# ubisoft/ubisoft-laforge-ZeroEGGS

Measured on AMD Instinct MI355X. Metric: train_frames_per_sec, higher is better.
Workload: dtype f32; 1 GPU; configs_v1.json nets (25.5M params, random-init), batch 32/GPU x 256-frame windows from synthetic 60fps 2-min clips, style example 384 frames, full train step (gather+fwd+loss+bwd+allreduce+RAdam); global_batch=32, window=256, parallelism=dp1

## Files before the change

### include/zeggs_hip.h

```cpp
#ifndef ZEGGS_HIP_H
#define ZEGGS_HIP_H
#include <stddef.h>
#include <stdint.h>

#ifdef __cplusplus
extern "C" {
#endif

int zeggs_version(void);
const char* zeggs_last_error(void);
int zeggs_set_option(const char* name, int value);
int zeggs_timing_ms(int which, float* ms);

int zeggs_gemm(const float* A, const float* B, float* C, const float* bias, int M, int N, int K,
               long sam, long sak, long sbk, long sbn, long scm, long scn, int nbatch, long bsA,
               long bsB, long bsC, float alpha, float beta, int act, void* stream);
int zeggs_gemm_tn_bias(const float* dy, long lddy, const float* x, long ldx, float* dW, long lddw, int M_contract, int N, int K,
                       float beta, float* db, void* stream);
int zeggs_gemm_direct_selftest(int big, int depth, int shield);
int zeggs_gemm_direct_state(int big, int depth, int shield);
int zeggs_gemm_direct_warm(void);
int zeggs_gemm_route(int direct, int shield, int depth, int reserve);
int zeggs_gemm_route_get(int* out4);
int zeggs_gemm_kbatch(const float* A, const float* B, float* C, int M, int N, int K, long sam, long sak, long sbk, long sbn,
// ... 136 lines not shown
int zeggs_decoder_bwd(const ZeggsDecDims*, const ZeggsDecParams*, const ZeggsDecStats*, const float* gaze,
                      const float* pose, const float* rpos, const float* rrot, const float* dpose,
                      const float* drpos, const float* drrot, const ZeggsDecGrads*, float* dspeech,
                      float* dstyle, void* ws, size_t ws_bytes, void* stream);
#define ZEGGS_STATUS_WORDS 4
#define ZEGGS_GAVE_UP_DECODE 1u
#define ZEGGS_GAVE_UP_TRAIN_FWD 2u
#define ZEGGS_GAVE_UP_BPTT 4u
#define ZEGGS_GAVE_UP_BATCH_FWD 8u
typedef struct {
  int prepared;
  int defer_wgrads;
  void* wgrad_stream;
  unsigned* status;
  int grads_zeroed;
} ZeggsDecCall;
int zeggs_decoder_fwd_ex(const ZeggsDecDims*, const ZeggsDecParams*, const ZeggsDecStats*, const float* pose0,
                         const float* rpos0, const float* rrot0, const float* gaze, const float* speech,
                         const float* style, float* pose, float* rpos, float* rrot, int training, void* ws,
                         size_t ws_bytes, void* stream, const ZeggsDecCall* call);
int zeggs_decoder_bwd_ex(const ZeggsDecDims*, const ZeggsDecParams*, const ZeggsDecStats*, const float* gaze,
                         const float* pose, const float* rpos, const float* rrot, const float* dpose,
                         const float* drpos, const float* drrot, const ZeggsDecGrads*, float* dspeech,
                         float* dstyle, void* ws, size_t ws_bytes, void* stream, const ZeggsDecCall* call);
int zeggs_decoder_fwd_state_ex(const ZeggsDecDims*, const ZeggsDecParams*, const ZeggsDecStats*, const float* pose0,
                               const float* rpos0, const float* rrot0, const float* gaze, const float* speech,
                               const float* style, float* pose, float* rpos, float* rrot, const float* h_in,
                               float* h_out, void* ws, size_t ws_bytes, void* stream, const ZeggsDecCall* call);
size_t zeggs_decoder_batch_workspace_bytes(const ZeggsDecDims*);
int zeggs_decoder_batch_prepare(const ZeggsDecDims*, const ZeggsDecParams*, const ZeggsDecStats*, void* ws, size_t ws_bytes,
// ... 201 lines not shown
```

### ubisoft-laforge-zeroeggs_amd/csrc/decoder.hip

```cpp
#include "../../include/zeggs_hip.h"
#include "common.h"
#include "gemm.h"
#include "kernels.h"
#include "dec_math.h"
#include "dec_prologue.h"
#include "decoder_ws.h"

int g_decoder_fast = 1;
int g_bwd_chunks = 1;
int g_tp_prologue = 1;
int g_wgrad_order = 0;

extern "C" int zeggs_persistent_state(int which ) {
  return g_sweep_kernels[which == 0 ? SWEEP_DECODE : which == 1 ? SWEEP_ROLLOUT : SWEEP_BPTT].state;
}

namespace {

__global__ void dec_init_k(ZeggsDecDims d, ZeggsDecStats st, const float* pose0, const float* rp0, const float* rr0,
                           const float* gaze, const float* style, float* pose, float* rpos, float* rrot,
                           float* cse_in, float* gin1, int GL) {
  dec_init_body(blockIdx.x, d, st, pose0, rp0, rr0, gaze, style, pose, rpos, rrot, cse_in, gin1, GL);
}

__global__ void dec_fill_cond_k(ZeggsDecDims d, const float* speech, const float* style, float* gin, int GL, int t0,
                                int nt, long slot_stride, int ring) {
// ... 117 lines not shown
    dst[b * ldd + c] = src[b * lds + off + c];
  }
}

__global__ void dec_scatter_cond_grad_k(ZeggsDecDims d, const float* DX, int XD, float* dspeech, float* dstyle) {
  const int XC = d.SP + (d.film ? 0 : d.ST);
  long n = (long)d.T * d.B * XC;
  for (long i = (long)blockIdx.x * blockDim.x + threadIdx.x; i < n; i += (long)gridDim.x * blockDim.x) {
    int c = (int)(i % XC);
    long r = i / XC;
    int b = (int)(r % d.B);
    int t = (int)(r / d.B);
    float v = t == 0 ? 0.f : DX[((long)t * d.B + b) * XD + d.PI + c];
    if (c < d.SP) dspeech[((long)b * d.T + t) * d.SP + c] = v;
    else dstyle[((long)b * d.T + t) * d.ST + (c - d.SP)] = v;
  }
}
__global__ void film_fwd_k(float* out, long ldo, const float* a, const float* gam, const float* bet, long ldg, int B,
                           int H) {
  long n = (long)B * H;
  for (long i = (long)blockIdx.x * blockDim.x + threadIdx.x; i < n; i += (long)gridDim.x * blockDim.x) {
    int u = (int)(i % H);
    long b = i / H;
    out[b * ldo + u] = a[i] * (1.f + gam[b * ldg + u]) + bet[b * ldg + u];
  }
}
__global__ void film_bwd_k(const float* g, long ldgr, const float* a, const float* gam, long ldg, float* dpre,
                           float* dgam, float* dbet, int B, int H) {
  long n = (long)B * H;
  for (long i = (long)blockIdx.x * blockDim.x + threadIdx.x; i < n; i += (long)gridDim.x * blockDim.x) {
// ... 311 lines not shown
    ZTRY(gemm_nn(w.DI0 + t * s3, 3 * H, P->w_ih0, H + XD, w.dGin, GL, B, 3 * H, H + XD, 0.f, s));
    if (d.film) {
      const long og = (long)t * B * 2 * H;
      hipLaunchKernelGGL(film_bwd_k, g1(sH), dim3(256), 0, s, w.dGin, (long)GL, w.A0 + o, w.GAM + og, (long)2 * H,
                         w.D0 + o, w.DGAM + og, w.DBET + og, B, H);
    } else {
      hipLaunchKernelGGL(elu_bwd_rows_k, g1(sH), dim3(256), 0, s, w.D0 + o, w.dGin, gin, B, H, GL);
    }
    float* dx = w.DX + (long)t * B * XD;
    hipLaunchKernelGGL(copy_cols_k, g1((long)B * XD), dim3(256), 0, s, dx, (long)XD, w.dGin, (long)GL, H, XD, B);
    ZLAUNCH_CHECK("dec_bwd_step");
    ZTRY(gemm_nn(w.D0 + o, H, P->l0_w, XD, dx, XD, B, H, XD, 1.f, s));
  }
  return 0;
}
int dec_cse_bwd(const DecCtx& c, const ZeggsDecGrads* G, float gb, hipStream_t gs) {
  const ZeggsDecParams* P = c.P; DecWs& w = c.w; hipStream_t s = c.s;
  const int B = c.d.B, H = c.d.H, CI = c.d.PI + c.d.ST;
  float* db = w.t0;
  float* da = w.t0 + (long)B * H;
  ZTRY(gemm_nn(w.dH0c, H, P->c2_w, H, db, H, B, H, H, 0.f, s));
  ZTRY(gemm_nn_actbwd(w.dH1c, H, P->c2_w + (long)H * H, H, db, H, B, H, H, 1.f, w.cse_b, H, ACT_ELU, s));
  ZTRY(gemm_nn_actbwd(db, H, P->c1_w, H, da, H, B, H, H, 0.f, w.cse_a, H, ACT_ELU, s));
  ZTRY(gemm_nn(da, H, P->c0_w, CI, w.t1, CI, B, H, CI, 0.f, s));
  if (gs) ZTRY(stream_fork(s, gs, 1));
  else gs = s;
  ZTRY(gemm_tn(w.dH0c, H, w.cse_b, H, G->c2_w, H, B, H, H, gb, gs));
  ZTRY(gemm_tn(w.dH1c, H, w.cse_b, H, G->c2_w + (long)H * H, H, B, H, H, gb, gs));
  ZTRY(k_colsum(G->c2_b, w.dH0c, B, H, H, gb, gs));
  ZTRY(k_colsum(G->c2_b + H, w.dH1c, B, H, H, gb, gs));
  ZTRY(gemm_tn(db, H, w.cse_a, H, G->c1_w, H, B, H, H, gb, gs));
  ZTRY(k_colsum(G->c1_b, db, B, H, H, gb, gs));
  ZTRY(gemm_tn(da, H, w.cse_in, CI, G->c0_w, CI, B, H, CI, gb, gs));
  return k_colsum(G->c0_b, da, B, H, H, gb, gs);
}
int dec_cond_grads(const DecCtx& c, float* dspeech, float* dstyle) {
  const ZeggsDecDims& d = c.d; const ZeggsDecParams* P = c.P; DecWs& w = c.w; hipStream_t s = c.s;
  const int B = d.B, T = d.T, H = d.H;
  hipLaunchKernelGGL(dec_scatter_cond_grad_k, g1((long)T * B * (d.SP + d.ST)), dim3(256), 0, s, d, w.DX, w.XD, dspeech, dstyle);
  if (d.film) {
    const long M1 = (long)(T - 1) * B, sg = (long)B * 2 * H, sS = (long)B * d.ST;
    ZTRY(gemm_nn(w.DGAM + sg, 2 * H, P->g_w, d.ST, w.dSTm + sS, d.ST, (int)M1, 2 * H, d.ST, 0.f, s));
    ZTRY(gemm_nn(w.DBET + sg, 2 * H, P->be_w, d.ST, w.dSTm + sS, d.ST, (int)M1, 2 * H, d.ST, 1.f, s));
    hipLaunchKernelGGL(style_grad_from_time_major_k, g1((long)T * B * d.ST), dim3(256), 0, s, d, w.dSTm, dstyle);
  }
  hipLaunchKernelGGL(add_style0_grad_k, g1((long)B * d.ST), dim3(256), 0, s, d, w.t1, dstyle);
  ZLAUNCH_CHECK("dec_bwd_tail");
  return 0;
}

}

extern "C" size_t zeggs_decoder_workspace_bytes(const ZeggsDecDims* d, int training) {
  Arena a(nullptr, 0);
  carve_dec(*d, training, a);
  return a.off + 256;
}

static int decoder_fwd_impl(const ZeggsDecDims* dp, const ZeggsDecParams* P, const ZeggsDecStats* st, const DecFwdIO& io,
                            int training, const float* h_in, float* h_out, void* ws, size_t ws_bytes, void* stream,
                            const ZeggsDecCall* call) {
  const ZeggsDecDims& d = *dp;
// ... 150 lines not shown
  Arena a(ws, ws_bytes);
  DecWs w = carve_dec(*dp, training, a);
  ZCHECK(a.ok() && w.chain, "chain_stamps: workspace too small or no fast path for these dims");
  ZCHECK(hipMemcpy(out, w.chain + 4 * 8 * 32 + 32, 16 * 2 * 16 * 8, hipMemcpyDeviceToHost) == hipSuccess, "copy failed");
  return 0;
}

extern "C" int zeggs_decoder_wgrads(const ZeggsDecDims* dp, const ZeggsDecGrads* G, void* ws, size_t ws_bytes, int what,
                                    void* stream) {
  const ZeggsDecDims& d = *dp;
  Arena a(ws, ws_bytes);
  DecWs w = carve_dec(d, 1, a);
  ZCHECK(a.ok(), "decoder wgrads: workspace too small (was the forward run with training=1?)");
  ZCHECK(d.T > 1, "decoder wgrads: T must be > 1");
  const bool fast_path = g_decoder_fast && dec_fast_supported(d);
  return dec_recurrent_wgrads(d, w, G, 1, d.T - 1, (what & 8) ? 1.f : 0.f, fast_path ? 1 : 0, (hipStream_t)stream, what & 5);
}
extern "C" int zeggs_decoder_prepare(const ZeggsDecDims* dp, const ZeggsDecParams* P, const ZeggsDecStats* st, void* ws,
                                     size_t ws_bytes, void* stream) {
  const ZeggsDecDims& d = *dp;
  hipStream_t s = (hipStream_t)stream;
  Arena a(ws, ws_bytes);
  DecWs w = carve_dec(d, 1, a);
  ZCHECK(a.ok(), "decoder prepare: workspace too small");
  const bool fast = g_decoder_fast && dec_fast_supported(d);
  const SweepKernel &tpk = g_sweep_kernels[SWEEP_ROLLOUT], &bpk = g_sweep_kernels[SWEEP_BPTT];
  if (!(fast && d.T > 1 && tpk.enabled && tpk.state == 1 && dec_tp_supported(d, w))) return 0;
  const DecCtx c{d, P, st, w, s};
  ZTRY(dec_tp_pack(c));
  ZTRY(dec_tp_zero(d, w, s));
  int mask = 1;
// ... 18 lines not shown
                                 float* dspeech, float* dstyle, void* ws, size_t ws_bytes, void* stream) {
  return zeggs_decoder_bwd_ex(dp, P, st, gaze, pose, rpos, rrot, dpose, drpos, drrot, G, dspeech, dstyle, ws, ws_bytes, stream,
                              nullptr);
}
extern "C" int zeggs_decoder_bwd_ex(const ZeggsDecDims* dp, const ZeggsDecParams* P, const ZeggsDecStats* st,
                                    const float* gaze, const float* pose, const float* rpos, const float* rrot,
                                    const float* dpose, const float* drpos, const float* drrot, const ZeggsDecGrads* G,
                                    float* dspeech, float* dstyle, void* ws, size_t ws_bytes, void* stream,
                                    const ZeggsDecCall* call) {
  const ZeggsDecDims& d = *dp;
  hipStream_t s = (hipStream_t)stream;
  const bool bwd_prepared = call && (call->prepared & 2);
  const int defer_wgrads = call ? call->defer_wgrads : 0;
  unsigned* status = call ? call->status : nullptr;
  const float gb = (call && call->grads_zeroed) ? 1.f : 0.f;
  ZCHECK(defer_wgrads == 0 || call->wgrad_stream != nullptr, "decoder bwd: defer_wgrads needs ZeggsDecCall.wgrad_stream");
  Arena a(ws, ws_bytes);
  DecWs w = carve_dec(d, 1, a);
  ZCHECK(a.ok(), "decoder bwd: workspace too small (was the forward run with training=1?)");
  const DecCtx c{d, P, st, w, s};
  const DecBwdIO io{gaze, pose, rpos, rrot, dpose, drpos, drrot};
  if (!bwd_prepared) ZTRY(dec_bwd_zero_state(c, true));
  ZCHECK(d.T > 1, "decoder bwd: T must be > 1");
  const bool fast_path = g_decoder_fast && dec_fast_supported(d);
  bool swept = false;
  SideStream* ss = nullptr;
  SweepKernel& bpk = g_sweep_kernels[SWEEP_BPTT];
  if (fast_path && dec_bp_supported(d, w) && bpk.may_run(s)) {
    ZTRY(dec_bp_run(c, io, bwd_prepared, bpk.status_arg(status)));
    ZTRY(bpk.settle(s, bp_errword(w), &swept));
    if (!swept) ZTRY(dec_bwd_zero_state(c, false));
  }
  if (!swept && fast_path) ZTRY(bwd_stage_sweep(c, io, G, gb, &ss));
  else if (!swept) ZTRY(bwd_generic_steps(c, io));
  const bool deferred = !ss && defer_wgrads && !stream_capturing(s);
  hipStream_t gs = deferred ? (hipStream_t)call->wgrad_stream : nullptr;
  const int what = deferred ? (defer_wgrads == 2 ? 1 : 5) | 2 : 7;
  if (deferred) ZTRY(stream_fork(s, gs, 0));
  if (!ss) ZTRY(dec_recurrent_wgrads(d, w, G, 1, d.T - 1, gb, fast_path ? 1 : 0, deferred ? gs : s, what));
  ZTRY(dec_cse_bwd(c, G, gb, gs));
  ZTRY(dec_cond_grads(c, dspeech, dstyle));
  if (ss) ZCHECK(hipStreamWaitEvent(s, ss->done, 0) == hipSuccess, "hipStreamWaitEvent failed");
  return 0;
}
```

### ubisoft-laforge-zeroeggs_amd/csrc/options.hip

```cpp
#include "../../include/zeggs_hip.h"
#include "common.h"
#include "decoder_ws.h"

extern int g_attn_bwd_one_launch, g_fused_attention;
extern int g_decoder_fast, g_bwd_chunks, g_tp_prologue, g_wgrad_order;
extern int g_stage_variant, g_timing, g_chain, g_sweep_graphs, g_launch_window;
extern int g_tp_tiles4, g_tp_dual;
extern int g_gemm_wg_target, g_gemm_streamk_wgs, g_gemm_mid_split, g_gemm_skinny, g_gemm_streamk, g_gemm_split_bf16;
extern int g_text_emit, g_text_passes;
extern int g_mel_mfma, g_mel_fft, g_mel_exact_log, g_loss_lds, g_ln_bwd4;
void zeggs_gemm_set_dma(int on), zeggs_gemm_set_direct(int mode, int wgs), zeggs_gemm_set_direct_depth(int d);
void zeggs_gemm_set_direct_shield(int on), zeggs_gemm_set_direct_reserve(int n), zeggs_gemm_set_asum(int on);

namespace {
enum Kind { AS_GIVEN, NONZERO, MIN0, MIN1, CALL };
struct Option { const char* name; int* target; Kind kind; int (*set)(int); };
int set_chain(int v) {
#ifndef ZEGGS_CHAIN
  if (v) { zeggs_set_error("option chain: the chained (run-ahead) stage launches lost to the persistent decode kernel and are "
                           "compiled in measurement builds only (-DZEGGS_CHAIN)"); return -1; }
#endif
  g_chain = v;
  return 0;
}
// ... 17 lines not shown
  {"gemm_direct", nullptr, CALL, [](int v) { zeggs_gemm_set_direct(v, -1); return 0; }},
  {"gemm_direct_wgs", nullptr, CALL, [](int v) { zeggs_gemm_set_direct(-1, v); return 0; }},
  {"gemm_direct_depth", nullptr, CALL, [](int v) { zeggs_gemm_set_direct_depth(v); return 0; }},
  {"gemm_direct_shield", nullptr, CALL, [](int v) { zeggs_gemm_set_direct_shield(v); return 0; }},
  {"gemm_direct_reserve", nullptr, CALL, [](int v) { zeggs_gemm_set_direct_reserve(v); return 0; }},
  {"gemm_asum", nullptr, CALL, [](int v) { zeggs_gemm_set_asum(v); return 0; }},
  {"gemm_skinny", &g_gemm_skinny, NONZERO},
  {"gemm_streamk", &g_gemm_streamk, NONZERO},
  {"fused_attention", &g_fused_attention, NONZERO},
  {"bwd_chunks", &g_bwd_chunks, MIN1},
  {"tp_tiles4", &g_tp_tiles4, NONZERO},
  {"tp_dual", &g_tp_dual, NONZERO},
  {"tp_prologue", &g_tp_prologue, NONZERO},
  {"loss_lds", &g_loss_lds, NONZERO},
  {"wgrad_order", &g_wgrad_order, AS_GIVEN},
  {"gemm_split_bf16", nullptr, CALL, [](int v) { g_gemm_split_bf16 = (v == 3 || v == 6 || v == 9) ? v : 0; return 0; }},
  {"poll_stagger", &g_poll_stagger, MIN0},
  {"poll_sleep", &g_poll_sleep, MIN0},
  {"persistent_spin", &g_persistent_spin, MIN0},
  {"ln_bwd4", &g_ln_bwd4, AS_GIVEN},
  {"mel_exact_log", &g_mel_exact_log, AS_GIVEN},
  {"text_emit", &g_text_emit, AS_GIVEN},
  {"text_passes", &g_text_passes, AS_GIVEN},
};
}

extern "C" int zeggs_set_option(const char* name, int value) {
  for (const Option& o : k_options) {
    if (strcmp(name, o.name) != 0) continue;
    if (o.kind == CALL) return o.set(value);
// ... 8 lines not shown
```

### ubisoft-laforge-zeroeggs_amd/zeggs/capi.py

```python
import ctypes as C
import os
import threading
from pathlib import Path

LIB_PATH = Path(os.environ.get("ZEGGS_LIB") or Path(__file__).resolve().parent / "libzeggs_hip.so")
OPTIONS = {}


class HipLibraryMissing(RuntimeError):
    pass


def _struct(name, fields):
    return type(name, (C.Structure,), {"_fields_": [(f, t) for t, names in fields for f in names.split()]})


def _ptr_struct(name, fields):
    return type(name, (C.Structure,), {"_fields_": [(f, C.c_void_p) for f in fields]})


SpeechDims = _struct("SpeechDims", [(C.c_int, "B T F H O KW"), (C.c_float, "dropout_p"), (C.c_uint64, "seed")])
LiveDims = _struct("LiveDims", [(C.c_int, "R F H O KW D feat_ld out_ld")])
LiveRow = _struct("LiveRow", [(C.c_long, "n_ring k0 last"), (C.c_int, "n_new n_out feat_off reserved")])
StyleDims = _struct("StyleDims", [(C.c_int, "B L C H E NH dropout"), (C.c_uint64, "seed")])
StyleGruDims = _struct("StyleGruDims", [(C.c_int, "B L C H O")])
DecDims = _struct("DecDims", [(C.c_int, "B T PI PO SP ST H"), (C.c_float, "dt"), (C.c_int, "film")])
DecCall = _struct("DecCall", [(C.c_int, "prepared defer_wgrads"), (C.c_void_p, "wgrad_stream status"), (C.c_int, "grads_zeroed")])
LossDims = _struct("LossDims", [(C.c_int, "B T J S"), (C.c_float, "dt")])
MelDims = _struct("MelDims", [(C.c_int, "n_fft hop n_mels fs"), (C.c_float, "fps min_clip"), (C.c_double, "pre_emph"), (C.c_int, "flags")])
AnimDims = _struct("AnimDims", [(C.c_int, "N J hips spine2 head"), (C.c_double, "dt"), (C.c_int, "order")])
BvhDims = _struct("BvhDims", [(C.c_int, "T J rebase"), (C.c_double * 3, "start_pos"), (C.c_double * 4, "start_rot"), (C.c_int, "order")])

SPEECH_FIELDS = ("w0", "b0", "w1", "b1", "w2", "b2")
STYLE_FIELDS = ("c0_w", "c0_b", "ln0_g", "ln0_b", "c4_w", "c4_b", "ln1_g", "ln1_b", "in_w", "in_b", "out_w", "out_b",
                "lna_g", "lna_b", "ff0_w", "ff0_b", "ff2_w", "ff2_b", "lnf_g", "lnf_b")
STYLE_GRU_FIELDS = ("c0_w", "c0_b", "c2_w", "c2_b", "w_ih", "w_hh", "b_ih", "b_hh", "w_ih_r", "w_hh_r", "b_ih_r",
                    "b_hh_r", "p_w", "p_b")
DEC_FIELDS = ("l0_w", "l0_b", "w_ih0", "w_hh0", "b_ih0", "b_hh0", "w_ih1", "w_hh1", "b_ih1", "b_hh1", "l2_w", "l2_b",
              "c0_w", "c0_b", "c1_w", "c1_b", "c2_w", "c2_b",
              "l3_w", "l3_b", "g_w", "g_b", "be_w", "be_b")
STATS_FIELDS = ("in_mean", "in_std", "out_mean", "out_std")
ANIM_OUT_FIELDS = ("root_pos", "root_rot", "root_vel", "root_vrt", "lpos", "lrot", "lvel", "lvrt", "ltxy", "cpos", "crot", "cvel",
# ... 275 lines not shown
```

### ubisoft-laforge-zeroeggs_amd/zeggs/engine.py

```python
import collections
import copy
import os
import warnings

import numpy as np
import torch

from . import ops
from .modules import kl_div_weight
from .optimizers import RAdam


class _IndexUploader:

    SLOTS = 4

    def __init__(self, device):
        self.device = torch.device(device)
        self.slots = [None] * self.SLOTS
        self.k = 0

    def __call__(self, arr):
        arr = np.ascontiguousarray(arr, dtype=np.int64)
        if self.device.type != "cuda":
# ... 423 lines not shown
                        self._last_sync_step = self._step_no
                        self._keep_prev, self._keep_next = self._keep_next, []
                        self._keep_prev.clear()
                        if not hit:
                            b["audio"].record_stream(self.aux_stream)
                        with torch.cuda.stream(self.aux_stream):
                            ops.fill_(self.flat_gx)
                            box["speech"] = self.se(b["audio"])
                    else:
                        box["speech"] = self.se(b["audio"])

                held = []
                example = self.style_type == "example"
                side = self.aux_stream is not None and self.wgrad_stream is not None
                hooked = example and side and type(getattr(self.st, "encoder", None)).__name__ == "StyleEncoderAttn"
                for bit, fn in ((1, launch_prepare), (2, launch_speech)):
                    if hooked and self.style_head_first & bit:
                        held.append(fn)
                    else:
                        fn()

                def release(inside=False):
                    ctx.after_style_head = None
                    self.head_first_releases += bool(held and inside)
                    with torch.enable_grad():
                        while held:
                            held.pop(0)()
                ctx.after_style_head = (lambda: release(True)) if held else None
                mu = logvar = None
                if example:
                    z, mu, logvar = self.st(b["example"], 1.0, eps=eps)
                else:
                    z = labels
                release()
                speech = box["speech"]
                style = ops.broadcast_time(z, T)
                if self.aux_stream is not None:
                    cur.wait_stream(self.aux_stream)
                    self._keep_next.append(speech)
                ev = lambda: torch.cuda.Event(enable_timing=True)
                if self.decoder_fwd_events is not None:
                    e0 = ev()
                    e0.record()
                self._dec_shape = (speech.shape[0], speech.shape[2], style.shape[2])
                pose, orp, orr = ops.decoder_core(self.de, b["pose0"], b["rpos0"], b["rrot0"], b["gaze"], speech, style,
                                                  ds.in_mean, ds.in_std, ds.out_mean, ds.out_std, self.dt)
                if self.decoder_fwd_events is not None:
                    e1 = ev()
                    e1.record()
                    self.decoder_fwd_events.append((e0, e1))
                klw = kl_div_weight(self.iteration) if mu is not None else 0.0
                loss, terms = ops.training_loss(pose, orp, orr, b["pose"], b["rpos"], b["rrot"], b["gaze"], self.parents,
                                                self.dt, mu, logvar, kl_weight=klw, gscale=1.0 / self.world,
                                                unit_grad=True, truth_ws=b.get("loss_ws"))
                if self.decoder_bwd_events is not None:
                    e2 = ev()
                    e2.record()
                loss.backward(self._one)
                if ctx.deferred_wgrads:
                    with torch.cuda.stream(self.aux_stream):
                        for evd, fn in ctx.deferred_wgrads:
                            self.aux_stream.wait_event(evd)
                            fn()
                    ctx.deferred_wgrads = []
                if self.decoder_bwd_events is not None:
                    e3 = ev()
                    e3.record()
                    self.decoder_bwd_events.append((e2, e3))
            done = True
        finally:
            ctx.after_style_head = None
            ctx.deferred_wgrads = []
            if not done:
                self.opt._early = []
                if self.wgrad_stream is not None:
                    torch.cuda.current_stream().wait_stream(self.wgrad_stream)
                ctx.release_wgrad_workspaces()
        if self.wgrad_stream is not None:
            torch.cuda.current_stream().wait_stream(self.wgrad_stream)
            ctx.release_wgrad_workspaces()
        if self.aux_stream is not None:
            torch.cuda.current_stream().wait_stream(self.aux_stream)
        if self.allreduce_events is not None:
            a0, a1 = torch.cuda.Event(enable_timing=True), torch.cuda.Event(enable_timing=True)
            a0.record()
        guarded_dp = self.status is not None and (self.world > 1 or self.force_allreduce)
        if guarded_dp and not self._flag_sent:
# ... 30 lines not shown
```

### ubisoft-laforge-zeroeggs_amd/zeggs/ops.py

```python
import ctypes as C

import numpy as np
import torch

from . import capi
from .capi import (DEC_FIELDS, SPEECH_FIELDS, STATS_FIELDS, STYLE_FIELDS, STYLE_GRU_FIELDS, DecCall, DecDims, DecPtrs,
                   DecStats, HipLibraryMissing, LiveDims, LiveRow, LossDims, MelRow, Seg, SpeechDims, SpeechPtrs, StyleDims,
                   StyleGruDims, StyleGruPtrs, StylePtrs, api)

_LIB_PATH = capi.LIB_PATH

COUNTERS = {}
STATUS_WORDS = 4
GAVE_UP = {1: "B=1 decode kernel", 2: "training rollout", 4: "BPTT sweep", 8: "batch decode sweep"}


def lib():
    return capi.raw()


def _check(rc, what):
    if rc != 0:
        raise RuntimeError(f"{what}: {lib().zeggs_last_error().decode()}")

# ... 43 lines not shown


class EngineContext:
    def __init__(self):
        self.direct_grads = False
        self.wgrad_stream = None
        self.status = None
        self.after_style_head = None
        self.after_decoder_backward = None
        self.decoder_grads_final = None
        self.prepared = None
        self.prepared_hits = 0
        self.wgrad_keepalive = []
        self.seed_rng = None
        self.gemm_route = None
        self.defer_style_wgrads = False
        self.deferred_wgrads = []

    def release_wgrad_workspaces(self):
        self.wgrad_keepalive.clear()

    def rng(self):
        return self.seed_rng if self.seed_rng is not None else _seed_rng


_DEFAULT_CTX = EngineContext()
_tls = threading.local()


def _route(ectx):
# ... 228 lines not shown
        ctx.d, ctx.ws = d, ws
        ctx.save_for_backward(*params)
        return out

    @staticmethod
    def backward(ctx, dout):
        params = list(ctx.saved_tensors)
        L = api()
        _route(ctx.ectx)
        grads, rets = _grad_targets(ctx.orig, params, ctx.ectx)
        P = _ptrs(StylePtrs, STYLE_FIELDS, params)
        G = _ptrs(StylePtrs, STYLE_FIELDS, grads)
        zeroed = int(ctx.ectx.direct_grads and all(r is None for r in rets))
        dout = _f32c(dout)
        ectx = ctx.ectx
        if ectx.defer_style_wgrads and zeroed:
            L.zeggs_style_encoder_bwd_part(ctx.d, P, dout, G, ctx.ws, ctx.ws.numel(), _stream(), zeroed, 1)
            ev = torch.cuda.Event()
            ev.record()
            d, ws, keep = ctx.d, ctx.ws, (params, grads, dout)

            def products():
                _route(ectx)
                L.zeggs_style_encoder_bwd_part(d, P, keep[2], G, ws, ws.numel(), _stream(), zeroed, 2)
            ectx.deferred_wgrads.append((ev, products))
            return (None, None, None, None, None, *rets)
        L.zeggs_style_encoder_bwd_ex(ctx.d, P, dout, G, ctx.ws, ctx.ws.numel(), _stream(), zeroed)
        return (None, None, None, None, None, *rets)


# ... 142 lines not shown
    if mask > 0:
        ectx.prepared = (_prepared_key(d, params, stats), ws, ev, int(mask))
    return int(mask)


def _warn_gave_up(bits, what, disabled=True):
    import warnings
    warnings.warn("zeggs: a persistent kernel gave up (" + ", ".join(n for b, n in GAVE_UP.items() if bits & b) +
                  "; another tenant on the GPU?); " + ("it is disabled for this process and " if disabled else "") + what +
                  " is redone on the stage kernels")


class _DecoderFn(torch.autograd.Function):
    @staticmethod
    def forward(ctx, pose0, rpos0, rrot0, gaze, speech, style, in_mean, in_std, out_mean, out_std, dt, H, grad_mode,
                *params):
        pose0, rpos0, rrot0, gaze, speech, style = (_f32c(t) for t in (pose0, rpos0, rrot0, gaze, speech, style))
        stats = [_f32c(t) for t in (in_mean, in_std, out_mean, out_std)]
        ectx = ctx.ectx = current()
        _route(ctx.ectx)
        ctx.orig = params
        params = [_f32c(t) for t in params]
        B, T, SP = speech.shape
        ST, PO = style.shape[2], pose0.shape[1]
        training = bool(grad_mode) and any(ctx.needs_input_grad)
        d = DecDims(B, T, PO + 3, PO, SP, ST, H, float(dt), 1 if len(params) == len(DEC_FIELDS) else 0)
        L = api()
        dev = pose0.device
        prep = ectx.prepared
        mask = 0
        if prep is not None and training and prep[0] == _prepared_key(d, params, stats):
            ectx.prepared = None
            _, ws, ev, mask = prep
            ectx.prepared_hits += 1
            torch.cuda.current_stream().wait_event(ev)
        else:
            _drop_prepared(ectx)
            ws = _ws(L.zeggs_decoder_workspace_bytes(d, int(training)), pose0.device)
# ... 20 lines not shown
        run()
        if own is not None:
            bits = int(own[0].item())
            if bits:
                _warn_gave_up(bits, "the rollout")
                for name in ("persistent", "train_persistent", "bwd_persistent"):
                    set_option(name, 0)
                fill_(own.view(torch.float32))
                call.prepared = 0
                run()
        global _LAST_DECODER_WS
        if _CHAIN_DIAGNOSTICS:
            _LAST_DECODER_WS = (d, int(training), ws)
        if training:
            ctx.d, ctx.ws = d, ws
            ctx.status, ctx.own_status = status, own is not None
            ctx.bwd_prepared = bool(mask & 2) and call.prepared != 0
            ctx.save_for_backward(gaze, pose, rpos, rrot, *stats, *params)
            ctx.set_materialize_grads(False)
        return pose, rpos, rrot

    @staticmethod
    def backward(ctx, dpose, drpos, drrot):
        gaze, pose, rpos, rrot, *rest = ctx.saved_tensors
        stats, params = rest[:4], rest[4:]
        d = ctx.d
        ectx = ctx.ectx
        _route(ectx)
        L = api()
        dev = pose.device
        z = lambda g, ref: fill_(torch.empty_like(ref)) if g is None else _f32c(g)
        dpose, drpos, drrot = z(dpose, pose), z(drpos, rpos), z(drrot, rrot)
        grads, rets = _grad_targets(ctx.orig, params, ectx)
        dspeech = torch.empty(d.B, d.T, d.SP, device=dev, dtype=torch.float32)
        dstyle = torch.empty(d.B, d.T, d.ST, device=dev, dtype=torch.float32)
        P = _ptrs(DecPtrs, DEC_FIELDS, params)
        G = _ptrs(DecPtrs, DEC_FIELDS, grads)
        S = _ptrs(DecStats, STATS_FIELDS, stats)
        direct = ectx.direct_grads and all(r is None for r in rets)
        side = ectx.wgrad_stream if direct and not torch.cuda.is_current_stream_capturing() else None
        after = ectx.after_decoder_backward
        chunked = side is not None and after is not None
        call = DecCall(2 if ctx.bwd_prepared else 0, 0 if side is None else (2 if chunked else 1),
                       side.cuda_stream if side is not None else None,
                       ctx.status.data_ptr() if ctx.status is not None else None, int(direct))

        def run():
            L.zeggs_decoder_bwd_ex(d, P, S, gaze, pose, rpos, rrot, dpose, drpos, drrot, G, dspeech, dstyle, ctx.ws, ctx.ws.numel(),
                                   _stream(), call)
        run()
        if ctx.own_status and not torch.cuda.is_current_stream_capturing():
            bits = int(ctx.status[0].item())
            if bits:
                _warn_gave_up(bits, "the BPTT sweep")
                for name in ("train_persistent", "bwd_persistent"):
                    set_option(name, 0)
                fill_(ctx.status.view(torch.float32))
                call.prepared = 0
                run()
        if side is not None:
            ectx.wgrad_keepalive.append(ctx.ws)
            if chunked:
                side.wait_stream(torch.cuda.current_stream())
                with torch.cuda.stream(side):
                    after(0)
                    L.zeggs_decoder_wgrads(d, G, ctx.ws, ctx.ws.numel(), 4 | 8, side.cuda_stream)
                    after(1)
            elif ectx.decoder_grads_final is not None:
                side.wait_stream(torch.cuda.current_stream())
                with torch.cuda.stream(side):
                    ectx.decoder_grads_final()
        elif after is not None and direct:
            after(None)
        return (None, None, None, None, dspeech, dstyle, None, None, None, None, None, None, None, *rets)


_LAST_DECODER_WS = None
_CHAIN_DIAGNOSTICS = False


def last_decoder_chain_errors():
    if _LAST_DECODER_WS is None:
        return 0
    d, training, ws = _LAST_DECODER_WS
    out = C.c_int(0)
    api().zeggs_decoder_chain_errors(d, training, ws, ws.numel(), C.byref(out))
    return int(out.value)


def decoder_core(dec, pose0, rpos0, rrot0, gaze, speech, style, in_mean, in_std, out_mean, out_std, dt):
    H = dec.recurrent_decoder.layer1.hidden_size
    return _DecoderFn.apply(pose0, rpos0, rrot0, gaze, speech, style, in_mean, in_std, out_mean, out_std, dt, H,
                            torch.is_grad_enabled(), *decoder_param_list(dec))


def decoder_rollout(dec, Z_root_pos, Z_root_rot, Z_root_vel, Z_root_vrt, Z_lpos, Z_ltxy, Z_lvel, Z_lvrt, gaze,
                    speech, style, in_mean, in_std, out_mean, out_std, dt):
    B, J = Z_lpos.shape[0], Z_lpos.shape[1]
    pose0 = torch.cat([Z_root_vel.reshape(B, -1), Z_root_vrt.reshape(B, -1), Z_lpos.reshape(B, -1),
                       Z_ltxy.reshape(B, -1), Z_lvel.reshape(B, -1), Z_lvrt.reshape(B, -1)], dim=1)
    pose, rpos, rrot = decoder_core(dec, pose0, Z_root_pos, Z_root_rot, gaze, speech, style, in_mean, in_std,
                                    out_mean, out_std, dt)
    T = pose.shape[1]
    return (rpos, rrot, pose[..., 0:3], pose[..., 3:6], pose[..., 6:6 + 3 * J].reshape(B, T, J, 3),
            pose[..., 6 + 3 * J:6 + 9 * J].reshape(B, T, J, 2, 3),
            pose[..., 6 + 9 * J:6 + 12 * J].reshape(B, T, J, 3),
            pose[..., 6 + 12 * J:6 + 15 * J].reshape(B, T, J, 3))

# ... 451 lines not shown
    rows = x.numel() // W
    vec = std if torch.is_tensor(std) and std.dim() > 0 else None
    sc = 1.0 if vec is not None else float(std)
    api().zeggs_normalize_rows(x, rows, W, W, mean, vec, sc, _stream())
    return x


_OPTIONS = capi.OPTIONS
_PERSISTENT_OPTION = ("persistent", "train_persistent", "bwd_persistent")


def _persistent_live(which):
    return _OPTIONS.get(_PERSISTENT_OPTION[which], 1) != 0 and api().zeggs_persistent_state(which) == 1


def set_option(name, value):
    global _CHAIN_DIAGNOSTICS, _LAST_DECODER_WS
    api().zeggs_set_option(name.encode(), int(value))
    _OPTIONS[name] = int(value)
    if name == "chain":
        _CHAIN_DIAGNOSTICS = bool(value)
        if not value:
            _LAST_DECODER_WS = None
```

Baseline: 495,600 frames/s.

## Fuse style-grad time reduction into decoder bwd and optionally hold tail wgrads

Example-style training now passes the per-clip style vector to the decoder instead of a broadcast [B,T,ST] tensor. The decoder backward sums the style gradient over time inside a new per-batch kernel, so it returns dz directly and skips the materialized dstyle tensor and the separate broadcast-backward reduction. The CSE backward is split into input-grad and weight-grad parts, and new options can run the head-side tail first or hold the decoder weight grads until the style encoder backward. This adds a new kernel and a new ABI field, and the hold path is opt-in.

```diff
diff --git a/include/zeggs_hip.h b/include/zeggs_hip.h
--- a/include/zeggs_hip.h
+++ b/include/zeggs_hip.h
@@ -174,6 +174,7 @@
   void* wgrad_stream;
   unsigned* status;
   int grads_zeroed;
+  float* dstyle_sum;
 } ZeggsDecCall;
 int zeggs_decoder_fwd_ex(const ZeggsDecDims*, const ZeggsDecParams*, const ZeggsDecStats*, const float* pose0,
                          const float* rpos0, const float* rrot0, const float* gaze, const float* speech,
diff --git a/ubisoft-laforge-zeroeggs_amd/csrc/decoder.hip b/ubisoft-laforge-zeroeggs_amd/csrc/decoder.hip
--- a/ubisoft-laforge-zeroeggs_amd/csrc/decoder.hip
+++ b/ubisoft-laforge-zeroeggs_amd/csrc/decoder.hip
@@ -10,6 +10,7 @@
 int g_bwd_chunks = 1;
 int g_tp_prologue = 1;
 int g_wgrad_order = 0;
+int g_tail_head_first = 0;
 
 extern "C" int zeggs_persistent_state(int which ) {
   return g_sweep_kernels[which == 0 ? SWEEP_DECODE : which == 1 ? SWEEP_ROLLOUT : SWEEP_BPTT].state;
@@ -157,6 +158,36 @@
     float v = t == 0 ? 0.f : DX[((long)t * d.B + b) * XD + d.PI + c];
     if (c < d.SP) dspeech[((long)b * d.T + t) * d.SP + c] = v;
     else dstyle[((long)b * d.T + t) * d.ST + (c - d.SP)] = v;
+  }
+}
+__global__ void __launch_bounds__(1024) dec_cond_grads_k(const float* DX, int XD, int PI, int SP, int ST, int B, int T,
+                                                         const float* dcse_in, float* dspeech, float* dstyle, float* dstyle_sum,
+                                                         int parts) {
+  extern __shared__ float sm[];
+  const int b = blockIdx.x, tid = threadIdx.x;
+  if (dstyle || dstyle_sum) {
+    if (tid < parts * ST) {
+      const int c = tid % ST, part = tid / ST;
+      float acc = 0.f;
+      for (int t = part; t < T; t += parts) {
+        const float v = t == 0 ? 0.f + dcse_in[(long)b * (PI + ST) + PI + c] : DX[((long)t * B + b) * XD + PI + SP + c];
+        if (dstyle) dstyle[((long)b * T + t) * ST + c] = v;
+        acc += v;
+      }
+      sm[tid] = acc;
+    }
+    if (dstyle_sum) {
+      __syncthreads();
+      if (tid < ST) {
+        float s = 0.f;
+        for (int q = 0; q < parts; ++q) s += sm[q * ST + tid];
+        dstyle_sum[(long)b * ST + tid] = s;
+      }
+    }
+  }
+  for (long i = tid; i < (long)T * SP; i += blockDim.x) {
+    const int c = (int)(i % SP), t = (int)(i / SP);
+    dspeech[((long)b * T + t) * SP + c] = t == 0 ? 0.f : DX[((long)t * B + b) * XD + PI + c];
   }
 }
 __global__ void film_fwd_k(float* out, long ldo, const float* a, const float* gam, const float* bet, long ldg, int B,
@@ -498,7 +529,7 @@
   }
   return 0;
 }
-int dec_cse_bwd(const DecCtx& c, const ZeggsDecGrads* G, float gb, hipStream_t gs) {
+int dec_cse_bwd_inputs(const DecCtx& c) {
   const ZeggsDecParams* P = c.P; DecWs& w = c.w; hipStream_t s = c.s;
   const int B = c.d.B, H = c.d.H, CI = c.d.PI + c.d.ST;
   float* db = w.t0;
@@ -506,9 +537,12 @@
   ZTRY(gemm_nn(w.dH0c, H, P->c2_w, H, db, H, B, H, H, 0.f, s));
   ZTRY(gemm_nn_actbwd(w.dH1c, H, P->c2_w + (long)H * H, H, db, H, B, H, H, 1.f, w.cse_b, H, ACT_ELU, s));
   ZTRY(gemm_nn_actbwd(db, H, P->c1_w, H, da, H, B, H, H, 0.f, w.cse_a, H, ACT_ELU, s));
-  ZTRY(gemm_nn(da, H, P->c0_w, CI, w.t1, CI, B, H, CI, 0.f, s));
-  if (gs) ZTRY(stream_fork(s, gs, 1));
-  else gs = s;
+  return gemm_nn(da, H, P->c0_w, CI, w.t1, CI, B, H, CI, 0.f, s);
+}
+int dec_cse_bwd_wgrads(const ZeggsDecDims& d, const DecWs& w, const ZeggsDecGrads* G, float gb, hipStream_t gs) {
+  const int B = d.B, H = d.H, CI = d.PI + d.ST;
+  const float* db = w.t0;
+  const float* da = w.t0 + (long)B * H;
   ZTRY(gemm_tn(w.dH0c, H, w.cse_b, H, G->c2_w, H, B, H, H, gb, gs));
   ZTRY(gemm_tn(w.dH1c, H, w.cse_b, H, G->c2_w + (long)H * H, H, B, H, H, gb, gs));
   ZTRY(k_colsum(G->c2_b, w.dH0c, B, H, H, gb, gs));
@@ -518,18 +552,31 @@
   ZTRY(gemm_tn(da, H, w.cse_in, CI, G->c0_w, CI, B, H, CI, gb, gs));
   return k_colsum(G->c0_b, da, B, H, H, gb, gs);
 }
-int dec_cond_grads(const DecCtx& c, float* dspeech, float* dstyle) {
+int cond_grads_launch(const float* DX, int XD, int PI, int SP, int ST, int B, int T, const float* dcse_in, float* dspeech,
+                      float* dstyle, float* dstyle_sum, hipStream_t s) {
+  ZCHECK(B >= 1 && T >= 1 && SP >= 0 && XD >= PI + SP + ST, "dec_cond_grads: bad dimensions");
+  ZCHECK(ST >= 1 && ST <= 1024, "dec_cond_grads: 1 <= ST <= 1024");
+  int parts = 1024 / ST;
+  if (parts > T) parts = T;
+  const int threads = (parts * ST + 63) / 64 * 64;
+  hipLaunchKernelGGL(dec_cond_grads_k, dim3(B), dim3(threads < 256 ? 256 : threads), threads * sizeof(float), s, DX, XD, PI, SP, ST, B,
+                     T, dcse_in, dspeech, dstyle, dstyle_sum, parts);
+  ZLAUNCH_CHECK("dec_cond_grads");
+  return 0;
+}
+int dec_cond_grads(const DecCtx& c, float* dspeech, float* dstyle, float* dstyle_sum) {
   const ZeggsDecDims& d = c.d; const ZeggsDecParams* P = c.P; DecWs& w = c.w; hipStream_t s = c.s;
   const int B = d.B, T = d.T, H = d.H;
-  hipLaunchKernelGGL(dec_scatter_cond_grad_k, g1((long)T * B * (d.SP + d.ST)), dim3(256), 0, s, d, w.DX, w.XD, dspeech, dstyle);
-  if (d.film) {
-    const long M1 = (long)(T - 1) * B, sg = (long)B * 2 * H, sS = (long)B * d.ST;
-    ZTRY(gemm_nn(w.DGAM + sg, 2 * H, P->g_w, d.ST, w.dSTm + sS, d.ST, (int)M1, 2 * H, d.ST, 0.f, s));
-    ZTRY(gemm_nn(w.DBET + sg, 2 * H, P->be_w, d.ST, w.dSTm + sS, d.ST, (int)M1, 2 * H, d.ST, 1.f, s));
-    hipLaunchKernelGGL(style_grad_from_time_major_k, g1((long)T * B * d.ST), dim3(256), 0, s, d, w.dSTm, dstyle);
-  }
+  if (!d.film) return cond_grads_launch(w.DX, w.XD, d.PI, d.SP, d.ST, B, T, w.t1, dspeech, dstyle, dstyle_sum, s);
+  ZCHECK(dstyle, "decoder bwd: the FiLM decoder needs the dstyle [B,T,ST] buffer");
+  hipLaunchKernelGGL(dec_scatter_cond_grad_k, g1((long)T * B * d.SP), dim3(256), 0, s, d, w.DX, w.XD, dspeech, dstyle);
+  const long M1 = (long)(T - 1) * B, sg = (long)B * 2 * H, sS = (long)B * d.ST;
+  ZTRY(gemm_nn(w.DGAM + sg, 2 * H, P->g_w, d.ST, w.dSTm + sS, d.ST, (int)M1, 2 * H, d.ST, 0.f, s));
+  ZTRY(gemm_nn(w.DBET + sg, 2 * H, P->be_w, d.ST, w.dSTm + sS, d.ST, (int)M1, 2 * H, d.ST, 1.f, s));
+  hipLaunchKernelGGL(style_grad_from_time_major_k, g1((long)T * B * d.ST), dim3(256), 0, s, d, w.dSTm, dstyle);
   hipLaunchKernelGGL(add_style0_grad_k, g1((long)B * d.ST), dim3(256), 0, s, d, w.t1, dstyle);
   ZLAUNCH_CHECK("dec_bwd_tail");
+  if (dstyle_sum) ZTRY(zeggs_sum_time(dstyle_sum, dstyle, B, T, d.ST, s));
   return 0;
 }
 
@@ -710,7 +757,10 @@
   ZCHECK(a.ok(), "decoder wgrads: workspace too small (was the forward run with training=1?)");
   ZCHECK(d.T > 1, "decoder wgrads: T must be > 1");
   const bool fast_path = g_decoder_fast && dec_fast_supported(d);
-  return dec_recurrent_wgrads(d, w, G, 1, d.T - 1, (what & 8) ? 1.f : 0.f, fast_path ? 1 : 0, (hipStream_t)stream, what & 5);
+  const float gb = (what & 8) ? 1.f : 0.f;
+  if (what & 7) ZTRY(dec_recurrent_wgrads(d, w, G, 1, d.T - 1, gb, fast_path ? 1 : 0, (hipStream_t)stream, what & 7));
+  if (what & 16) ZTRY(dec_cse_bwd_wgrads(d, w, G, gb, (hipStream_t)stream));
+  return 0;
 }
 extern "C" int zeggs_decoder_prepare(const ZeggsDecDims* dp, const ZeggsDecParams* P, const ZeggsDecStats* st, void* ws,
                                      size_t ws_bytes, void* stream) {
@@ -759,6 +809,7 @@
   const int defer_wgrads = call ? call->defer_wgrads : 0;
   unsigned* status = call ? call->status : nullptr;
   const float gb = (call && call->grads_zeroed) ? 1.f : 0.f;
+  float* dstyle_sum = call ? call->dstyle_sum : nullptr;
   ZCHECK(defer_wgrads == 0 || call->wgrad_stream != nullptr, "decoder bwd: defer_wgrads needs ZeggsDecCall.wgrad_stream");
   Arena a(ws, ws_bytes);
   DecWs w = carve_dec(d, 1, a);
@@ -780,11 +831,27 @@
   else if (!swept) ZTRY(bwd_generic_steps(c, io));
   const bool deferred = !ss && defer_wgrads && !stream_capturing(s);
   hipStream_t gs = deferred ? (hipStream_t)call->wgrad_stream : nullptr;
+  const bool held = deferred && defer_wgrads == 3;
   const int what = deferred ? (defer_wgrads == 2 ? 1 : 5) | 2 : 7;
+  const bool head_first = g_tail_head_first != 0 && !ss;
+  if (head_first) {
+    ZTRY(dec_cse_bwd_inputs(c));
+    ZTRY(dec_cond_grads(c, dspeech, dstyle, dstyle_sum));
+  }
   if (deferred) ZTRY(stream_fork(s, gs, 0));
-  if (!ss) ZTRY(dec_recurrent_wgrads(d, w, G, 1, d.T - 1, gb, fast_path ? 1 : 0, deferred ? gs : s, what));
-  ZTRY(dec_cse_bwd(c, G, gb, gs));
-  ZTRY(dec_cond_grads(c, dspeech, dstyle));
+  if (!ss && !held) ZTRY(dec_recurrent_wgrads(d, w, G, 1, d.T - 1, gb, fast_path ? 1 : 0, deferred ? gs : s, what));
+  if (!head_first) {
+    ZTRY(dec_cse_bwd_inputs(c));
+    if (deferred) ZTRY(stream_fork(s, gs, 1));
+  }
+  if (!held) ZTRY(dec_cse_bwd_wgrads(d, w, G, gb, deferred ? gs : s));
+  if (!head_first) ZTRY(dec_cond_grads(c, dspeech, dstyle, dstyle_sum));
   if (ss) ZCHECK(hipStreamWaitEvent(s, ss->done, 0) == hipSuccess, "hipStreamWaitEvent failed");
   return 0;
 }
+
+extern "C" int zeggs_dec_cond_grads(const float* DX, int XD, int PI, int SP, int ST, int B, int T, const float* dcse_in,
+                                    float* dspeech, float* dstyle, float* dstyle_sum, void* stream) {
+  ZCHECK(DX && dcse_in && dspeech, "dec_cond_grads: DX, dcse_in and dspeech are required");
+  return cond_grads_launch(DX, XD, PI, SP, ST, B, T, dcse_in, dspeech, dstyle, dstyle_sum, (hipStream_t)stream);
+}
diff --git a/ubisoft-laforge-zeroeggs_amd/csrc/options.hip b/ubisoft-laforge-zeroeggs_amd/csrc/options.hip
--- a/ubisoft-laforge-zeroeggs_amd/csrc/options.hip
+++ b/ubisoft-laforge-zeroeggs_amd/csrc/options.hip
@@ -3,7 +3,7 @@
 #include "decoder_ws.h"
 
 extern int g_attn_bwd_one_launch, g_fused_attention;
-extern int g_decoder_fast, g_bwd_chunks, g_tp_prologue, g_wgrad_order;
+extern int g_decoder_fast, g_bwd_chunks, g_tp_prologue, g_wgrad_order, g_tail_head_first;
 extern int g_stage_variant, g_timing, g_chain, g_sweep_graphs, g_launch_window;
 extern int g_tp_tiles4, g_tp_dual;
 extern int g_gemm_wg_target, g_gemm_streamk_wgs, g_gemm_mid_split, g_gemm_skinny, g_gemm_streamk, g_gemm_split_bf16;
@@ -55,6 +55,7 @@
   {"tp_prologue", &g_tp_prologue, NONZERO},
   {"loss_lds", &g_loss_lds, NONZERO},
   {"wgrad_order", &g_wgrad_order, AS_GIVEN},
+  {"tail_head_first", &g_tail_head_first, AS_GIVEN},
   {"gemm_split_bf16", nullptr, CALL, [](int v) { g_gemm_split_bf16 = (v == 3 || v == 6 || v == 9) ? v : 0; return 0; }},
   {"poll_stagger", &g_poll_stagger, MIN0},
   {"poll_sleep", &g_poll_sleep, MIN0},
diff --git a/ubisoft-laforge-zeroeggs_amd/zeggs/capi.py b/ubisoft-laforge-zeroeggs_amd/zeggs/capi.py
--- a/ubisoft-laforge-zeroeggs_amd/zeggs/capi.py
+++ b/ubisoft-laforge-zeroeggs_amd/zeggs/capi.py
@@ -25,7 +25,8 @@
 StyleDims = _struct("StyleDims", [(C.c_int, "B L C H E NH dropout"), (C.c_uint64, "seed")])
 StyleGruDims = _struct("StyleGruDims", [(C.c_int, "B L C H O")])
 DecDims = _struct("DecDims", [(C.c_int, "B T PI PO SP ST H"), (C.c_float, "dt"), (C.c_int, "film")])
-DecCall = _struct("DecCall", [(C.c_int, "prepared defer_wgrads"), (C.c_void_p, "wgrad_stream status"), (C.c_int, "grads_zeroed")])
+DecCall = _struct("DecCall", [(C.c_int, "prepared defer_wgrads"), (C.c_void_p, "wgrad_stream status"), (C.c_int, "grads_zeroed"),
+                              (C.c_void_p, "dstyle_sum")])
 LossDims = _struct("LossDims", [(C.c_int, "B T J S"), (C.c_float, "dt")])
 MelDims = _struct("MelDims", [(C.c_int, "n_fft hop n_mels fs"), (C.c_float, "fps min_clip"), (C.c_double, "pre_emph"), (C.c_int, "flags")])
 AnimDims = _struct("AnimDims", [(C.c_int, "N J hips spine2 head"), (C.c_double, "dt"), (C.c_int, "order")])
diff --git a/ubisoft-laforge-zeroeggs_amd/zeggs/engine.py b/ubisoft-laforge-zeroeggs_amd/zeggs/engine.py
--- a/ubisoft-laforge-zeroeggs_amd/zeggs/engine.py
+++ b/ubisoft-laforge-zeroeggs_amd/zeggs/engine.py
@@ -461,6 +461,8 @@
                 example = self.style_type == "example"
                 side = self.aux_stream is not None and self.wgrad_stream is not None
                 hooked = example and side and type(getattr(self.st, "encoder", None)).__name__ == "StyleEncoderAttn"
+                ctx.hold_wgrads = bool(hooked and not overlap and ops.option("tail_head_first") == 2)
+                ctx.held_wgrads = None
                 for bit, fn in ((1, launch_prepare), (2, launch_speech)):
                     if hooked and self.style_head_first & bit:
                         held.append(fn)
@@ -481,7 +483,7 @@
                     z = labels
                 release()
                 speech = box["speech"]
-                style = ops.broadcast_time(z, T)
+                style = z if example else ops.broadcast_time(z, T)
                 if self.aux_stream is not None:
                     cur.wait_stream(self.aux_stream)
                     self._keep_next.append(speech)
@@ -489,9 +491,9 @@
                 if self.decoder_fwd_events is not None:
                     e0 = ev()
                     e0.record()
-                self._dec_shape = (speech.shape[0], speech.shape[2], style.shape[2])
+                self._dec_shape = (speech.shape[0], speech.shape[2], style.shape[-1])
                 pose, orp, orr = ops.decoder_core(self.de, b["pose0"], b["rpos0"], b["rrot0"], b["gaze"], speech, style,
-                                                  ds.in_mean, ds.in_std, ds.out_mean, ds.out_std, self.dt)
+                                                  ds.in_mean, ds.in_std, ds.out_mean, ds.out_std, self.dt, style_broadcast=example)
                 if self.decoder_fwd_events is not None:
                     e1 = ev()
                     e1.record()
@@ -504,6 +506,9 @@
                     e2 = ev()
                     e2.record()
                 loss.backward(self._one)
+                if ctx.held_wgrads is not None:
+                    release, ctx.held_wgrads = ctx.held_wgrads, None
+                    release()
                 if ctx.deferred_wgrads:
                     with torch.cuda.stream(self.aux_stream):
                         for evd, fn in ctx.deferred_wgrads:
@@ -518,6 +523,7 @@
         finally:
             ctx.after_style_head = None
             ctx.deferred_wgrads = []
+            ctx.hold_wgrads, ctx.held_wgrads = False, None
             if not done:
                 self.opt._early = []
                 if self.wgrad_stream is not None:
diff --git a/ubisoft-laforge-zeroeggs_amd/zeggs/ops.py b/ubisoft-laforge-zeroeggs_amd/zeggs/ops.py
--- a/ubisoft-laforge-zeroeggs_amd/zeggs/ops.py
+++ b/ubisoft-laforge-zeroeggs_amd/zeggs/ops.py
@@ -81,6 +81,9 @@
         self.wgrad_keepalive = []
         self.seed_rng = None
         self.gemm_route = None
+        self.hold_wgrads = False
+        self.held_wgrads = None
+        self.held_releases = 0
         self.defer_style_wgrads = False
         self.deferred_wgrads = []
 
@@ -339,6 +342,10 @@
         zeroed = int(ctx.ectx.direct_grads and all(r is None for r in rets))
         dout = _f32c(dout)
         ectx = ctx.ectx
+        release, ectx.held_wgrads = ectx.held_wgrads, None
+        if release is not None:
+            ectx.held_releases += 1
+            release()
         if ectx.defer_style_wgrads and zeroed:
             L.zeggs_style_encoder_bwd_part(ctx.d, P, dout, G, ctx.ws, ctx.ws.numel(), _stream(), zeroed, 1)
             ev = torch.cuda.Event()
@@ -511,7 +518,7 @@
 class _DecoderFn(torch.autograd.Function):
     @staticmethod
     def forward(ctx, pose0, rpos0, rrot0, gaze, speech, style, in_mean, in_std, out_mean, out_std, dt, H, grad_mode,
-                *params):
+                style_broadcast, *params):
         pose0, rpos0, rrot0, gaze, speech, style = (_f32c(t) for t in (pose0, rpos0, rrot0, gaze, speech, style))
         stats = [_f32c(t) for t in (in_mean, in_std, out_mean, out_std)]
         ectx = ctx.ectx = current()
@@ -519,6 +526,9 @@
         ctx.orig = params
         params = [_f32c(t) for t in params]
         B, T, SP = speech.shape
+        if style_broadcast:
+            z, style = style, torch.empty(B, T, style.shape[1], device=style.device, dtype=torch.float32)
+            api().zeggs_broadcast_time(style, z, B, T, z.shape[1], _stream())
         ST, PO = style.shape[2], pose0.shape[1]
         training = bool(grad_mode) and any(ctx.needs_input_grad)
         d = DecDims(B, T, PO + 3, PO, SP, ST, H, float(dt), 1 if len(params) == len(DEC_FIELDS) else 0)
@@ -569,6 +579,7 @@
             _LAST_DECODER_WS = (d, int(training), ws)
         if training:
             ctx.d, ctx.ws = d, ws
+            ctx.style_broadcast = bool(style_broadcast)
             ctx.status, ctx.own_status = status, own is not None
             ctx.bwd_prepared = bool(mask & 2) and call.prepared != 0
             ctx.save_for_backward(gaze, pose, rpos, rrot, *stats, *params)
@@ -588,7 +599,11 @@
         dpose, drpos, drrot = z(dpose, pose), z(drpos, rpos), z(drrot, rrot)
         grads, rets = _grad_targets(ctx.orig, params, ectx)
         dspeech = torch.empty(d.B, d.T, d.SP, device=dev, dtype=torch.float32)
-        dstyle = torch.empty(d.B, d.T, d.ST, device=dev, dtype=torch.float32)
+        want_style = ctx.needs_input_grad[5]
+        dz = torch.empty(d.B, d.ST, device=dev, dtype=torch.float32) if want_style and ctx.style_broadcast else None
+        dstyle = None
+        if d.film or (want_style and dz is None):
+            dstyle = torch.empty(d.B, d.T, d.ST, device=dev, dtype=torch.float32)
         P = _ptrs(DecPtrs, DEC_FIELDS, params)
         G = _ptrs(DecPtrs, DEC_FIELDS, grads)
         S = _ptrs(DecStats, STATS_FIELDS, stats)
@@ -596,9 +611,11 @@
         side = ectx.wgrad_stream if direct and not torch.cuda.is_current_stream_capturing() else None
         after = ectx.after_decoder_backward
         chunked = side is not None and after is not None
-        call = DecCall(2 if ctx.bwd_prepared else 0, 0 if side is None else (2 if chunked else 1),
+        hold = side is not None and not chunked and ectx.hold_wgrads
+        call = DecCall(2 if ctx.bwd_prepared else 0, 0 if side is None else (2 if chunked else 3 if hold else 1),
                        side.cuda_stream if side is not None else None,
-                       ctx.status.data_ptr() if ctx.status is not None else None, int(direct))
+                       ctx.status.data_ptr() if ctx.status is not None else None, int(direct),
+                       dz.data_ptr() if dz is not None else None)
 
         def run():
             L.zeggs_decoder_bwd_ex(d, P, S, gaze, pose, rpos, rrot, dpose, drpos, drrot, G, dspeech, dstyle, ctx.ws, ctx.ws.numel(),
@@ -615,7 +632,18 @@
                 run()
         if side is not None:
             ectx.wgrad_keepalive.append(ctx.ws)
-            if chunked:
+            if hold:
+                ws, final = ctx.ws, ectx.decoder_grads_final
+
+                def release(keep=(params, grads)):
+                    _route(ectx)
+                    side.wait_stream(torch.cuda.current_stream())
+                    with torch.cuda.stream(side):
+                        L.zeggs_decoder_wgrads(d, G, ws, ws.numel(), 1 | 2 | 4 | 16 | (8 if direct else 0), side.cuda_stream)
+                        if final is not None:
+                            final()
+                ectx.held_wgrads = release
+            elif chunked:
                 side.wait_stream(torch.cuda.current_stream())
                 with torch.cuda.stream(side):
                     after(0)
@@ -627,7 +655,8 @@
                     ectx.decoder_grads_final()
         elif after is not None and direct:
             after(None)
-        return (None, None, None, None, dspeech, dstyle, None, None, None, None, None, None, None, *rets)
+        return (None, None, None, None, dspeech, dz if ctx.style_broadcast else dstyle if want_style else None, None, None, None, None,
+                None, None, None, None, *rets)
 
 
 _LAST_DECODER_WS = None
@@ -643,10 +672,10 @@
     return int(out.value)
 
 
-def decoder_core(dec, pose0, rpos0, rrot0, gaze, speech, style, in_mean, in_std, out_mean, out_std, dt):
+def decoder_core(dec, pose0, rpos0, rrot0, gaze, speech, style, in_mean, in_std, out_mean, out_std, dt, style_broadcast=False):
     H = dec.recurrent_decoder.layer1.hidden_size
     return _DecoderFn.apply(pose0, rpos0, rrot0, gaze, speech, style, in_mean, in_std, out_mean, out_std, dt, H,
-                            torch.is_grad_enabled(), *decoder_param_list(dec))
+                            torch.is_grad_enabled(), bool(style_broadcast), *decoder_param_list(dec))
 
 
 def decoder_rollout(dec, Z_root_pos, Z_root_rot, Z_root_vel, Z_root_vrt, Z_lpos, Z_ltxy, Z_lvel, Z_lvrt, gaze,
@@ -1128,6 +1157,13 @@
     return _OPTIONS.get(_PERSISTENT_OPTION[which], 1) != 0 and api().zeggs_persistent_state(which) == 1
 
 
+_OPTION_DEFAULTS = {"tail_head_first": 0}
+
+
+def option(name):
+    return _OPTIONS.get(name, _OPTION_DEFAULTS[name])
+
+
 def set_option(name, value):
     global _CHAIN_DIAGNOSTICS, _LAST_DECODER_WS
     api().zeggs_set_option(name.encode(), int(value))
```

Measured after the change: 496,200 frames/s (median of 6 runs). About the same (+0.1%).
